# pbs-plus/pbs-plus

Measured on AMD Instinct MI355X. Metric: GiB/s ingested through CDC+SHA-256, higher is better.
Workload: dtype u32

## Files before the change

pbs_plus_amd/csrc/kernels.h:

```cpp
#pragma once

#include <hip/hip_runtime.h>
#include <stdint.h>

#include "../../include/pbsgpu.h"

namespace pbsk {

constexpr int kWindow = 64;

struct ScanParams {
    const uint8_t *data_al;
    uint32_t lead;
    uint64_t nbytes;
    uint64_t ntiles;
    uint32_t tile_bytes;
    const uint32_t *table_rot;
    uint32_t thr;
    uint32_t cap;
    uint32_t *tile_cnt;
    uint32_t *tile_slots;
    unsigned long long *tile_queue;
    uint32_t tiles_per_wave;
    uint32_t shared_chip;
// ... 159 lines not shown
    const uint4 *ldesc;
    uint32_t lmask;
    uint32_t long_bytes;
    const uint4 *sdesc;
    uint32_t smask;
    uint32_t short_bytes;
    uint32_t short_room;
    RingCtl *ctl;
    uint8_t *cells;
    uint32_t *pending;
    unsigned long long *free_fifo;
    uint32_t free_mask;
    const uint32_t *heartbeat;
    unsigned long long idle_ticks;
    uint32_t poll_mask;
    uint32_t xp;
    uint32_t long_spill;
    uint32_t xp_pairs;
    uint32_t long_lo;
};
constexpr int kHbBeat = 0, kHbIntent = 16, kHbCommitted = 17, kHbClaim = 32, kHbRoundsEnq = 33;
constexpr uint32_t kRingProbeSteps = 4096;


enum : int { kRsNcand = 0, kRsNrec = 1, kRsMaxcnt = 2, kRsNlong = 3, kRsNshort = 4, kRsShortRoom = 5, kRsTileq = 6 , kRsNmain = 8, kRsCount = 10 };

struct RingPage {
    uint64_t phys_off;
    uint64_t logical;
    uint32_t valid;
    uint32_t slot;
    uint32_t phys;
    uint32_t seg;
    uint64_t fill_seed;
    uint64_t fill_off;
    uint32_t fill_kind;
    uint32_t do_fill;
    const struct FillPiece *fill_tab;
    uint32_t fill_ntab;
    uint32_t prev_phys;
};
struct FillPiece {
    uint64_t dst_off, len, src_off, seed;
};
struct RingSeg {
    uint32_t slot;
    uint32_t first_page;
    uint32_t npages;
    uint32_t final;
    uint64_t new_end;
    uint32_t reset;
    uint32_t pad;
    uint64_t origin;
};
constexpr uint64_t kRingMaxStream = 1ull << kRingOffBits;
constexpr uint32_t kRingPT = 512;
struct RingStreamState {
    uint64_t c;
    uint64_t end;
    uint64_t ecand;
    uint32_t pad[2];
    uint32_t pt[kRingPT];
};
struct RingRoundStatus {
    uint32_t seq;
    uint32_t nrec;
    uint32_t ncand;
    uint32_t error;
    uint32_t tail;
    uint32_t pad[3];
    unsigned long long probe[6];
    uint32_t phase_ticks[6];
};
static_assert(sizeof(RingRoundStatus) == 104, "host slot: 128 bytes (ring.cpp: input_stride)");
struct RingRound {
    uint8_t *arena;
    uint32_t page_bytes, stride, tile_bytes, tpp;
// ... 7 lines not shown
    uint32_t seq;
    uint32_t cell_base, cell_cap, cell_mask;
    uint32_t scan_blocks;
    RingRoundStatus *status;
    RingStreamState *streams;
    RingSource q;
    uint4 *desc_w;
    uint4 *ldesc_w;
    uint4 *sdesc_w;
    unsigned long long *tile_queue;
    uint32_t *scalars;
    uint32_t *tile_cnt, *tile_off, *tile_slots, *scan_tmp;
    uint64_t *dense;
    uint64_t dense_cap;
    pbsgpu_segment *segs;
    uint32_t *seg_cnt, *seg_off;
    pbsgpu_record *recs;
    uint64_t rec_cap;
    uint64_t *seg_newc;
    uint32_t *seg_open;
    uint64_t *seg_ecand_in;
    uint64_t *seg_ecand;
    const uint64_t *sugg;
    const uint32_t *sugg_idx;
    uint64_t sugg_feed;
    uint32_t sugg_abs;
    uint32_t pad0;
    const uint32_t *seg_rec_base;
};
struct RingStage {
    const uint8_t *src;
    uint8_t *dst;
    uint32_t off[4], len[4];
    const RingPage *pages_host;
};
hipError_t launch_ring_round(const RingRound &r, int num_cus, hipStream_t st, hipStream_t fill_st = nullptr,
                             hipEvent_t fill_ev = nullptr, hipStream_t scan_st = nullptr, hipEvent_t scan_ev = nullptr,
                             const RingStage *stage = nullptr);
hipError_t launch_ring_service(const RingSource &q, unsigned workgroups, hipStream_t st, bool dense = false);
hipError_t launch_ring_service_xp(const RingSource &q, unsigned workgroups, hipStream_t st);
hipError_t launch_ring_service_lanes(const RingSource &q, unsigned workgroups, hipStream_t st, bool dense);
hipError_t launch_ring_stop(RingCtl *ctl, hipStream_t st);
hipError_t launch_ring_reset(RingCtl *ctl, hipStream_t st);

struct PackItem {
    uint64_t src_off;
    uint64_t dst_off;
    uint64_t len;
    uint32_t kind;
    uint32_t pad;
};
hipError_t launch_pack(const uint8_t *src_base, uint8_t *dst, const PackItem *items, uint32_t nitems, hipStream_t st);

}
```

pbs_plus_amd/csrc/ring.cpp:

```cpp
#include <chrono>
#include <cstdio>
#include <cstdlib>
#include <thread>

#include "ring_internal.h"

using namespace pbse;

namespace {

double now_ms() {
    return std::chrono::duration<double, std::milli>(std::chrono::steady_clock::now().time_since_epoch()).count();
}

uint32_t pow2_at_least(uint64_t v) {
    uint32_t p = 1;
    while (p < v && p < (1u << 31)) p <<= 1;
    return p;
}

volatile uint32_t *hb_words(const pbsgpu_ring *r) { return r->heartbeat.as<volatile uint32_t>(); }

void ring_service_ended(pbsgpu_ring *r) {
    if (r->svc == SvcState::Stopped) return;
// ... 135 lines not shown
int ring_start_service(pbsgpu_ring *r, bool force = false) {
    if (r->svc == SvcState::Running) return PBSGPU_OK;
    if (r->svc == SvcState::Stopping && r->parked_for_flush) {
        HIPCHK(hipStreamSynchronize(r->ss));
        ring_service_ended(r);
    }
    const uint32_t park_gen = service_park_generation(r->eng->device);
    if (r->svc == SvcState::Stopped && !force && park_gen != 0 && park_gen != r->park_grace_gen) {
        const double t = now_ms();
        if (r->park_wait_t0 == 0) r->park_wait_t0 = t;
        if (t - r->park_wait_t0 < 250.0) return PBSGPU_OK;
        r->park_grace_gen = park_gen;
    }
    r->park_wait_t0 = 0;
    if (r->svc == SvcState::Stopping) {
        HIPCHK(hipStreamWaitEvent(r->cs, r->ev_svc1, 0));
        HIPCHK(pbsk::launch_ring_reset(r->ctl.as<pbsk::RingCtl>(), r->cs));
        HIPCHK(hipEventRecord(r->ev_reset, r->cs));
    } else {
        service_started(r->eng->device);
    }
    r->svc = SvcState::Running;
    ring_adapt_split(r);
    r->defer_t0 = 0;
    hb_words(r)[pbsk::kHbClaim] = r->tail_seen;
    CHK(ring_launch_services(r));
    r->svc_t0 = now_ms();
    r->svc_bytes0 = r->st.bytes_enqueued - r->deferred_bytes;
    r->deferred_bytes = 0;
    r->st.service_launches++;
    return PBSGPU_OK;
}

int ring_enqueue_round(pbsgpu_ring *r, bool *did) {
    *did = false;
    pbsgpu_engine *e = r->eng;
    if (r->error != PBSGPU_OK) return r->error;
    bool any = false, any_final = false;
    size_t ready = 0;
    for (auto &s : r->slots) {
        if (!s.open) continue;
        any |= !s.ready.empty() || s.zero_final;
        any_final |= s.zero_final || (!s.ready.empty() && s.ready.back().final);
        ready += s.ready.size();
    }
    if (!any) return PBSGPU_OK;
    {
        size_t inflight = 0;
        for (auto &ri : r->rounds) inflight += ri.reaped ? 0 : 1;
        if (inflight > 0 && !any_final && ready < r->min_round_pages) return PBSGPU_OK;
        if (inflight >= r->max_inflight) return PBSGPU_OK;
    }
    int in = -1;
    for (uint32_t i = 0; i < kRingInputs; ++i)
        if (!r->input_busy[i]) { in = (int)i; break; }
    if (in < 0) return PBSGPU_OK;
    {
        const uint64_t oldest = r->rounds.empty() ? r->cell_cursor : r->rounds.front().cell_base;
        if (r->cell_cursor + r->rec_cap - oldest > r->ncells) return PBSGPU_OK;
    }
    pbsk::RingPage *pg = r->in_pages((uint32_t)in);
    pbsk::RingSeg *sg = r->in_segs((uint32_t)in);
    uint32_t *recbase = r->in_recbase((uint32_t)in);
    uint32_t *suggidx = r->in_suggidx((uint32_t)in);
    uint32_t np = 0, ns = 0;
    uint64_t cells_needed = 0, new_bytes = 0;
    RoundInfo ri;
    std::vector<hipEvent_t> deps;
    std::vector<uint64_t> sugg;
    const uint32_t minsz = std::min(e->effmin, e->cfg.min);
    const uint64_t feed = e->sugg_feed.load(std::memory_order_relaxed);
    const uint64_t look = feed > 1 ? (uint64_t)e->cfg.max : 0;
    uint32_t streams_waiting = 0;
    for (auto &s : r->slots) streams_waiting += (s.open && !s.ready.empty()) ? 1u : 0u;
    const uint32_t round_cap = (r->svc == SvcState::Stopped || streams_waiting < 2)
                                   ? r->round_pages
                                   : std::max(std::min(r->round_pages, r->min_round_pages), r->round_pages / 2);
    for (uint32_t si = 0; si < r->slots.size() && np < round_cap; ++si) {
        StreamSlot &s = r->slots[si];
        if (!s.open || (s.ready.empty() && !s.zero_final)) continue;
        pbsk::RingSeg g{};
        g.slot = si;
        g.first_page = np;
        g.reset = s.fresh ? 1u : 0u;
        g.origin = s.origin;
        const uint64_t end_old = s.bytes_enqueued;
        uint64_t end = end_old;
        uint32_t take = 0;
        while (!s.ready.empty() && take < kPagesPerStreamRound && np < round_cap) {
            const PageReq &q = s.ready.front();
            pbsk::RingPage p{};
            p.phys = q.phys;
            p.phys_off = (uint64_t)q.phys * r->stride + 128u;
            p.logical = ((uint64_t)si << pbsk::kRingOffBits) | (q.k * r->page_bytes);
            p.valid = q.valid;
            p.slot = si;
            p.seg = ns;
            p.do_fill = q.do_fill ? 1u : 0u;
            p.fill_seed = q.seed;
            p.fill_off = q.fill_off;
            p.fill_kind = q.kind;
            p.fill_tab = q.tab;
            p.fill_ntab = q.ntab;
            p.prev_phys = (q.k > 0 && s.last_phys >= 0) ? (uint32_t)s.last_phys : 0xffffffffu;
            s.last_phys = (int64_t)q.phys;
            pg[np++] = p;
            if (q.dep) deps.push_back(q.dep);
            end += q.valid;
            new_bytes += q.valid;
            if (q.final) g.final = 1;
            s.ready.pop_front();
            ++take;
        }
        if (s.zero_final && s.ready.empty()) {
            g.final = 1;
            s.zero_final = false;
        }
        g.npages = take;
        g.new_end = end;
        s.bytes_enqueued = end;
        s.fresh = false;
        if (g.final) {
            s.final_enqueued = true;
            ri.finals.push_back(si);
        }
        suggidx[ns] = (uint32_t)sugg.size();
        {
            const uint64_t lower = end_old > e->cfg.max ? end_old - e->cfg.max : 0;
            while (!s.sugg.empty() && s.sugg.front() < lower) s.sugg.pop_front();
            for (uint64_t b : s.sugg) {
                if (b > end + look) break;
                sugg.push_back(b);
            }
        }
        recbase[ns] = (uint32_t)cells_needed;
        cells_needed += ((uint64_t)take * r->page_bytes + e->cfg.max) / minsz + 2;
        sg[ns++] = g;
    }
    if (ns == 0) return PBSGPU_OK;
    suggidx[ns] = (uint32_t)sugg.size();
// ... 72 lines not shown
    rr.recs = r->recs.as<pbsgpu_record>();
    rr.rec_cap = r->rec_cap;
    rr.seg_newc = r->seg_newc.as<uint64_t>();
    rr.seg_open = r->seg_open.as<uint32_t>();
    rr.seg_ecand_in = r->seg_ecand_in.as<uint64_t>();
    rr.seg_ecand = r->seg_ecand.as<uint64_t>();
    rr.sugg = sugg_dev;
    rr.sugg_idx = sugg_dev ? suggidx : nullptr;
    rr.sugg_feed = feed;
    rr.sugg_abs = e->sugg_feed_abs.load(std::memory_order_relaxed);
    rr.seg_rec_base = recbase;
    std::atomic_thread_fence(std::memory_order_release);
    bool defer = r->defer_service;
    if (!defer && r->svc == SvcState::Stopped && r->lone_defer_ms > 0 && !any_final &&
        np >= std::max<uint32_t>(1, r->round_pages / 2)) {
        const uint64_t lanes_worth = (uint64_t)r->sha_cus * (r->dense_service ? 256u : 128u) * (uint64_t)e->cfg.avg;
        const double t = now_ms();
        if (r->defer_t0 == 0) r->defer_t0 = t;
        defer = t - r->defer_t0 < r->lone_defer_ms && r->deferred_bytes + new_bytes < lanes_worth;
    }
    if (!defer) {
        const int st = ring_start_service(r);
        if (st != PBSGPU_OK) return fail(st);
        rr.q = r->source();
    }
    if (r->svc == SvcState::Stopped) r->deferred_bytes += new_bytes;
    if (r->svc == SvcState::Stopped) rr.scan_blocks = (uint32_t)std::max(1, e->num_cus);
    else if (r->ps && rr.scan_blocks > 8) rr.scan_blocks -= 1;
    hipStream_t scan_st = r->ps ? r->ps : r->cs;
    for (hipEvent_t ev : deps)
        if (hipStreamWaitEvent(scan_st, ev, 0) != hipSuccess) return fail(PBSGPU_E_HIP);
    for (hipEvent_t ev : deps) ring_event_put(r, ev);
    deps.clear();
    if (r->ps && r->ctl_used[set])
        if (hipStreamWaitEvent(r->ps, r->ev_ctl[set], 0) != hipSuccess) return fail(PBSGPU_E_HIP);
    {
        const bool fill_serial = r->fill_serial;
        pbsk::RingStage stg{};
        if (r->stage_inputs) {
            const uint8_t *hb = r->in((uint32_t)in);
            uint8_t *db = r->in_dev((uint32_t)in);
            stg.src = hb;
            stg.dst = db;
            stg.off[0] = (uint32_t)r->in_pages_off;   stg.len[0] = np * (uint32_t)sizeof(pbsk::RingPage);
            stg.off[1] = (uint32_t)r->in_segs_off;    stg.len[1] = ns * (uint32_t)sizeof(pbsk::RingSeg);
            stg.off[2] = (uint32_t)r->in_recbase_off; stg.len[2] = (ns + 1u) * 4u;
            stg.off[3] = (uint32_t)r->in_suggidx_off; stg.len[3] = rr.sugg_idx ? (ns + 1u) * 4u : 0u;
            stg.pages_host = pg;
            auto mirror = [&](const void *hp) { return db + (reinterpret_cast<const uint8_t *>(hp) - hb); };
            rr.pages = reinterpret_cast<const pbsk::RingPage *>(mirror(pg));
            rr.segs_in = reinterpret_cast<const pbsk::RingSeg *>(mirror(sg));
            rr.seg_rec_base = reinterpret_cast<const uint32_t *>(mirror(recbase));
            if (rr.sugg_idx) rr.sugg_idx = reinterpret_cast<const uint32_t *>(mirror(suggidx));
        }
        const hipError_t he = pbsk::launch_ring_round(rr, e->num_cus, r->cs, fill_serial ? nullptr : r->fs, r->ev_fill[in], r->ps,
                                                      r->ps ? r->ev_scan[in] : nullptr, r->stage_inputs ? &stg : nullptr);
        if (he != hipSuccess) {
            g_last_hip_error.store((int)he);
            return fail(PBSGPU_E_HIP);
        }
    }
    if (r->ps) {
        if (hipEventRecord(r->ev_ctl[set], r->cs) != hipSuccess) return fail(PBSGPU_E_HIP);
        r->ctl_used[set] = true;
        r->scan_set ^= 1u;
    }
    r->input_busy[in] = true;
    ri.new_bytes = new_bytes;
    r->ready_bytes -= new_bytes;
    r->inflight_bytes += new_bytes;
    r->rounds.push_back(std::move(ri));
    r->st.rounds++;
    r->st.bytes_enqueued += new_bytes;
    r->st.pages_enqueued += np;
    *did = true;
    return PBSGPU_OK;
}

int ring_take_page(pbsgpu_ring *r, uint32_t *phys) {
    if (r->backlog_limit && r->svc == SvcState::Running) {
        const int32_t behind = (int32_t)(r->tail_seen - hb_words(r)[pbsk::kHbClaim]) - 256;
        double wait = (double)r->ready_bytes + (double)r->inflight_bytes;
        if (behind > 0 && r->pub_positions) wait += (double)behind * ((double)r->pub_bytes / (double)r->pub_positions);
        if (wait > (double)r->backlog_limit) return PBSGPU_E_BUSY;
    }
    if (r->free_pages.empty()) ring_reap_free(r);
    if (r->free_pages.empty()) return PBSGPU_E_BUSY;
    *phys = r->free_pages.back();
    r->free_pages.pop_back();
// ... 211 lines not shown
            arena_bytes = fr > (12ull << 30) ? fr - (8ull << 30) : fr / 2;
        }
        r->npages = (uint32_t)std::min<uint64_t>(arena_bytes / r->stride, 65534);
        {
            const uint64_t lim = (4ull << 20) * std::min(e->effmin, e->cfg.min) / r->page_bytes;
            if (r->npages > lim) r->npages = (uint32_t)std::max<uint64_t>(lim, 4);
        }
        if (r->npages < 4) return PBSGPU_E_INVALID;
        r->max_streams = o.max_streams ? o.max_streams : 64;
        if (r->max_streams > 4096) return PBSGPU_E_INVALID;
        int sha = o.sha_cus ? (int)o.sha_cus : std::max(1, e->num_cus - e->num_cus / 4);
        int xp = o.express_cus == PBSGPU_RING_OFF ? 0 : (int)o.express_cus;
        if (o.express_cus == 0 && !o.sha_cus && e->num_cus >= 128) xp = 16;
        xp = std::min(xp, std::max(0, e->num_cus / 2));
        if (xp && !o.sha_cus) sha = std::max(1, sha - xp);
        const int svc_max = std::max(2, e->num_cus - e->num_cus / 4 + (e->num_cus >= 64 ? 8 : 0));
        if (sha + xp > svc_max) sha = std::max(1, svc_max - xp);
        r->xp_cus = (uint32_t)xp;
        r->sha_cus = (uint32_t)std::min(std::max(sha, 1), std::max(1, e->num_cus - 1 - xp));
        r->lanes_cus = std::min<uint32_t>(o.lanes_cus, r->sha_cus * 3u / 4u);
        r->sha_cus -= r->lanes_cus;
        r->short_bytes = o.short_bytes ? (uint32_t)std::min<uint64_t>(o.short_bytes, e->cfg.max) : (uint32_t)((uint64_t)e->cfg.avg * 3 / 2);
        r->svc_cus = r->sha_cus + r->xp_cus + r->lanes_cus;
        r->split_auto = xp > 0 && !o.sha_cus && !o.express_cus && r->svc_cus >= 96 && !(o.flags & PBSGPU_RING_F_NO_SPLIT_AUTO);
        r->round_pages = o.round_pages ? o.round_pages : 256;
        r->round_pages = std::min(r->round_pages, r->npages);
        r->min_round_pages = o.min_round_pages ? std::max(1u, std::min(o.min_round_pages, std::max(1u, r->round_pages / 4)))
                                               : std::max(1u, r->round_pages / 4);
        r->backlog_limit = o.backlog_mib < 0 ? 0 : o.backlog_mib > 0 ? (uint64_t)(o.backlog_mib * 1048576.0)   : (uint64_t)(r->sha_cus + r->lanes_cus) << 27;
        r->backlog_auto = o.backlog_mib == 0;
        if (o.max_inflight) r->max_inflight = std::min<uint32_t>(std::max(1u, o.max_inflight), kRingInputs);
        r->autopark_ms = std::max(0.0, o.autopark_ms);
        r->defer_service = (o.flags & PBSGPU_RING_F_DEFER_SERVICE) != 0;
        r->fill_serial = (o.flags & PBSGPU_RING_F_FILL_SERIAL) != 0;
        r->dense_service = (o.flags & PBSGPU_RING_F_DENSE_SERVICE) != 0;
        r->dense_lanes = (o.flags & PBSGPU_RING_F_DENSE_LANES) != 0;
        r->tier_tag = (o.flags & PBSGPU_RING_F_TIER_TAG) != 0;
        r->lone_defer_ms = o.lone_defer_ms < 0 ? 0.0 : o.lone_defer_ms > 0 ? o.lone_defer_ms : 25.0;
        r->idle_timeout_s = o.idle_timeout_s;
        r->opt_long_lo = o.long_lo_bytes;
        r->opt_long_spill = o.long_spill;
        r->opt_poll_every = o.poll_every;
        const double lambda = 3.0 * r->tile_bytes / ((double)e->cfg.mask + 1.0);
        uint32_t capv = 8;
        while (capv < 4.0 * lambda + 16.0) capv <<= 1;
        r->cap = std::min<uint32_t>(std::max<uint32_t>(capv * 2, r->tile_bytes / 128), r->tile_bytes);
        const uint64_t ntiles = (uint64_t)r->round_pages * r->tpp;
        if (ntiles * r->cap >= (1ull << 32)) return PBSGPU_E_INVALID;
        const uint32_t minsz = std::min(e->effmin, e->cfg.min);
        r->dense_cap = ntiles * r->cap;
        r->rec_cap = ((uint64_t)r->round_pages * r->page_bytes + (uint64_t)r->max_streams * e->cfg.max) / minsz +
                     4ull * r->max_streams + 64;
        const uint64_t resident_chunks = (uint64_t)r->npages * r->page_bytes / minsz + 2ull * r->npages + r->rec_cap;
        r->qslots = pow2_at_least(2 * resident_chunks + 4096);
        r->ncells = pow2_at_least(4 * resident_chunks + 4 * r->rec_cap);
        r->nfree = pow2_at_least(4ull * r->npages + 64);

        CHK(r->arena.ensure((size_t)r->npages * r->stride + 512));
        CHK(r->ctl.ensure(256));
        CHK(r->probe.ensure(128));
        CHK(r->streams.ensure((size_t)r->max_streams * sizeof(pbsk::RingStreamState)));
        CHK(r->pending.ensure((size_t)r->npages * 4 + 64));
        CHK(r->desc.ensure((size_t)r->qslots * 32));
        r->long_bytes = r->xp_cus ? (long_bytes_hint ? long_bytes_hint : (uint32_t)((uint64_t)e->cfg.max * 13 / 16)) : 0;
        r->long_lo_auto = long_bytes_hint == 0;
        if (o.long_bytes) r->long_bytes = o.long_bytes == PBSGPU_RING_OFF ? 0u : o.long_bytes;
        if (r->xp_cus && r->long_bytes == 0) r->xp_cus = 0;
// ... 98 lines not shown
    return ring_create_internal(e, opt, true, out);
}

int pbsgpu_ring_quiesce(pbsgpu_ring *r) {
    if (!r) return PBSGPU_E_INVALID;
    CHK(set_device(r->eng));
    ring_heartbeat(r);
    if (r->defer_service && r->svc == SvcState::Stopped) {
        HIPCHK(hipStreamSynchronize(r->cs));
        HIPCHK(pbsk::launch_ring_stop(r->ctl.as<pbsk::RingCtl>(), r->cs));
        HIPCHK(hipEventRecord(r->ev_reset, r->cs));
        CHK(ring_launch_services(r));
        service_started(r->eng->device);
        r->svc = SvcState::Running;
        r->st.service_launches++;
        HIPCHK(hipStreamSynchronize(r->ss));
        ring_service_ended(r);
        HIPCHK(hipStreamSynchronize(r->cs));
        r->svc_bytes0 = r->st.bytes_enqueued;
        ring_reap_free(r);
        ring_reap_rounds(r);
        return r->error;
    }
    if (r->svc == SvcState::Stopped && r->deferred_bytes > 0) {
        CHK(ring_start_service(r, true));
    }
    if (r->svc == SvcState::Running) {
        CHK(ring_service_check(r, false));
        if (r->svc == SvcState::Running) HIPCHK(pbsk::launch_ring_stop(r->ctl.as<pbsk::RingCtl>(), r->cs));
    }
    HIPCHK(hipStreamSynchronize(r->cs));
    if (r->svc != SvcState::Stopped) {
        HIPCHK(hipStreamSynchronize(r->ss));
        HIPCHK(hipStreamSynchronize(r->fs));
        ring_service_ended(r);
    }
    ring_reap_free(r);
    ring_reap_rounds(r);
    return r->error;
}

int pbsgpu_ring_park(pbsgpu_ring *r) {
    if (!r) return PBSGPU_E_INVALID;
    CHK(set_device(r->eng));
    ring_heartbeat(r);
    CHK(ring_park(r));
    return r->error;
}

void pbsgpu_ring_destroy(pbsgpu_ring *r) {
    if (!r) return;
    pbsgpu_engine *e = r->eng;
    if (e) {
        (void)hipSetDevice(e->device);
        if (r->cs && r->ss) (void)pbsgpu_ring_quiesce(r);
        if (r->svc != SvcState::Stopped) {
            r->svc = SvcState::Stopped;
            service_ended(r->eng->device);
        }
        if (r->ss) (void)hipStreamDestroy(r->ss);
        if (r->xs) (void)hipStreamDestroy(r->xs);
        if (r->ev_xsvc1) (void)hipEventDestroy(r->ev_xsvc1);
        if (r->ls) (void)hipStreamDestroy(r->ls);
        if (r->ev_lsvc1) (void)hipEventDestroy(r->ev_lsvc1);
        if (r->cs) (void)hipStreamDestroy(r->cs);
        if (r->ps) (void)hipStreamDestroy(r->ps);
        if (r->fs) (void)hipStreamDestroy(r->fs);
        for (auto ev : r->ev_scan)
            if (ev) (void)hipEventDestroy(ev);
        for (auto ev : r->ev_ctl)
            if (ev) (void)hipEventDestroy(ev);
        for (auto ev : r->ev_fill)
            if (ev) (void)hipEventDestroy(ev);
        for (hipEvent_t ev : {r->ev_reset, r->ev_svc0, r->ev_svc1})
            if (ev) (void)hipEventDestroy(ev);
        for (auto &s : r->slots)
            for (auto &q : s.ready)
                if (q.dep) r->ev_pool.push_back(q.dep);
        for (auto ev : r->ev_pool) (void)hipEventDestroy(ev);
        for (DevBuf *b : {&r->arena, &r->ctl, &r->probe, &r->streams, &r->pending, &r->desc, &r->ldesc, &r->sdesc, &r->scalars, &r->tile_cnt, &r->tile_off,
                          &r->tile_slots, &r->tile_cnt2, &r->tile_slots2, &r->tileq, &r->scan_tmp, &r->dense, &r->segs, &r->seg_cnt, &r->seg_off, &r->recs, &r->seg_newc,
                          &r->seg_open, &r->seg_ecand_in, &r->seg_ecand, &r->inputs_dev})
            b->release();
        r->cells.release();
        r->heartbeat.release();
        r->free_fifo.release();
        r->inputs.release();
        for (auto &b : r->sugg_in) b.release();
// ... 208 lines not shown
    StreamSlot &s = r->slots[stream];
    if (s.final_committed) return PBSGPU_E_STATE;
    if (!s.sugg.empty() && offset < s.sugg.back()) return PBSGPU_E_INVALID;
    s.sugg.push_back(offset);
    return PBSGPU_OK;
}

int pbsgpu_ring_fill(pbsgpu_ring *r, uint32_t stream, uint64_t seed, uint32_t kind, uint64_t nbytes, int final,
                     uint64_t *taken) {
    if (!r || !taken || stream >= r->slots.size() || !r->slots[stream].open || kind > 4) return PBSGPU_E_INVALID;
    StreamSlot &s = r->slots[stream];
    *taken = 0;
    if (s.final_committed || s.reserved >= 0) return PBSGPU_E_STATE;
    if (r->error != PBSGPU_OK) return r->error;
    if (s.bytes_committed + nbytes > pbsk::kRingMaxStream) return PBSGPU_E_INVALID;
    if (nbytes == 0) {
        if (final) {
            s.zero_final = true;
            s.final_committed = true;
        }
        return PBSGPU_OK;
    }
    while (*taken < nbytes) {
        const uint64_t n = std::min<uint64_t>(r->page_bytes, nbytes - *taken);
        const bool last = (*taken + n == nbytes);
        if (n < r->page_bytes && !(last && final)) break;
        uint32_t phys = 0;
        if (ring_take_page(r, &phys) != PBSGPU_OK) break;
        PageReq q;
        q.phys = phys;
        q.k = s.next_k++;
        q.valid = (uint32_t)n;
        q.final = last && final;
        q.do_fill = true;
        q.seed = seed;
        q.kind = kind;
        q.fill_off = s.bytes_committed;
        if (r->hold) r->held.assign(stream, q.k, q.phys);
        s.ready.push_back(q);
        r->ready_bytes += n;
        s.bytes_committed += n;
        *taken += n;
        if (q.final) s.final_committed = true;
    }
    return PBSGPU_OK;
}

int pbsgpu_ring_fill_pieces(pbsgpu_ring *r, uint32_t stream, const pbsgpu_fill_piece *pieces, uint32_t npieces, uint64_t nbytes,
                            int final, uint64_t *taken) {
    if (!r || !taken || stream >= r->slots.size() || !r->slots[stream].open) return PBSGPU_E_INVALID;
    static_assert(sizeof(pbsgpu_fill_piece) == sizeof(pbsk::FillPiece), "piece layout");
    StreamSlot &s = r->slots[stream];
    *taken = 0;
    if (s.final_committed || s.reserved >= 0) return PBSGPU_E_STATE;
    if (r->error != PBSGPU_OK) return r->error;
    if (pieces) {
        if (npieces == 0 || s.bytes_committed != 0) return PBSGPU_E_INVALID;
        uint64_t pos = 0;
        for (uint32_t i = 0; i < npieces; ++i) {
            if (pieces[i].dst_off != pos || pieces[i].len == 0 || ((pieces[i].dst_off | pieces[i].len | pieces[i].src_off) & 15u))
                return PBSGPU_E_INVALID;
            pos += pieces[i].len;
        }
        CHK(r->piece_tab[stream].ensure(std::max<size_t>((size_t)npieces * sizeof(pbsk::FillPiece), 4096)));
        std::memcpy(r->piece_tab[stream].p, pieces, (size_t)npieces * sizeof(pbsk::FillPiece));
        r->piece_n[stream] = npieces;
    }
    const uint32_t nt = r->piece_n[stream];
    if (nt == 0) return PBSGPU_E_STATE;
    const pbsk::FillPiece *tab = r->piece_tab[stream].as<pbsk::FillPiece>();
    const uint64_t total = tab[nt - 1].dst_off + tab[nt - 1].len;
    if (s.bytes_committed + nbytes > total || s.bytes_committed + nbytes > pbsk::kRingMaxStream) return PBSGPU_E_INVALID;
    if (nbytes == 0) {
        if (final) {
            s.zero_final = true;
            s.final_committed = true;
        }
        return PBSGPU_OK;
    }
    while (*taken < nbytes) {
        const uint64_t n = std::min<uint64_t>(r->page_bytes, nbytes - *taken);
        const bool last = (*taken + n == nbytes);
        if (n < r->page_bytes && !(last && final)) break;
        uint32_t phys = 0;
        if (ring_take_page(r, &phys) != PBSGPU_OK) break;
        PageReq q;
        q.phys = phys;
        q.k = s.next_k++;
        q.valid = (uint32_t)n;
        q.final = last && final;
        q.do_fill = true;
        q.kind = 5;
        q.tab = tab;
        q.ntab = nt;
        q.fill_off = s.bytes_committed;
        if (r->hold) r->held.assign(stream, q.k, q.phys);
        s.ready.push_back(q);
        r->ready_bytes += n;
        s.bytes_committed += n;
        *taken += n;
        if (q.final) s.final_committed = true;
    }
    return PBSGPU_OK;
}

int pbsgpu_ring_pump(pbsgpu_ring *r) {
    if (!r) return PBSGPU_E_INVALID;
    CHK(set_device(r->eng));
    ring_heartbeat(r);
    CHK(ring_service_check(r, false));
    if (r->svc == SvcState::Stopping) {
        const hipError_t q = hipEventQuery(r->ev_svc1);
        if (q == hipSuccess) ring_service_ended(r);
        else (void)hipGetLastError();
    }
    ring_reap_free(r);
    ring_reap_rounds(r);
    if (r->svc == SvcState::Running) {
        const uint32_t gen = service_park_generation(r->eng->device);
        if (gen && gen != r->park_gen_seen) {
            r->park_gen_seen = gen;
            CHK(ring_park(r));
            if (r->svc == SvcState::Stopping) r->parked_for_flush = true;
        }
    }
    bool any_round = false;
    for (int i = 0; i < 4; ++i) {
        bool did = false;
        CHK(ring_enqueue_round(r, &did));
        if (!did) break;
        any_round = true;
    }
    if (!r->defer_service && r->svc == SvcState::Stopped && r->deferred_bytes > 0) {
        bool waiting = false;
        for (auto &s : r->slots) waiting |= s.open && !s.ready.empty();
        const uint64_t lanes_worth = (uint64_t)r->sha_cus * (r->dense_service ? 256u : 128u) * (uint64_t)r->eng->cfg.avg;
        if ((!any_round && !waiting) || now_ms() - r->defer_t0 >= r->lone_defer_ms || r->deferred_bytes >= lanes_worth)
            CHK(ring_start_service(r));
    }
    if (r->autopark_ms > 0 && r->svc == SvcState::Running) {
        if (ring_idle(r)) {
            const double t = now_ms();
// ... 138 lines not shown
```

pbs_plus_amd/csrc/ring_internal.h:

```cpp
#pragma once

#include <deque>
#include <mutex>
#include <vector>

#include "engine_internal.h"
#include "hold.h"

namespace pbse {

constexpr uint32_t kRingInputs = 16;
constexpr uint32_t kPagesPerStreamRound = 256;

struct PageReq {
    uint32_t phys = 0;
    uint64_t k = 0;
    uint32_t valid = 0;
    bool final = false;
    bool do_fill = false;
    uint64_t seed = 0, fill_off = 0;
    uint32_t kind = 0;
    const pbsk::FillPiece *tab = nullptr;
    uint32_t ntab = 0;
    hipEvent_t dep = nullptr;
};

struct CellRef {
    uint32_t cell;
    uint32_t round_idx;
};

struct StreamSlot {
    bool open = false;
    bool fresh = true;
    uint64_t next_k = 0;
    uint64_t bytes_committed = 0;
    uint64_t bytes_enqueued = 0;
    bool final_committed = false, final_enqueued = false, final_done = false;
    bool zero_final = false;
    int64_t reserved = -1;
    int64_t last_phys = -1;
    std::deque<PageReq> ready;
    std::deque<CellRef> cells;
    uint64_t records_out = 0;
    uint64_t polled_end = 0;
    bool reported = false;
    uint64_t origin = 0;
    std::deque<uint64_t> sugg;
    void *owner = nullptr;
};

struct RoundInfo {
    uint32_t seq = 0;
    uint32_t input = 0;
    uint64_t cell_base = 0;
    uint32_t cell_cap = 0;
// ... 23 lines not shown
    pbse::DevBuf arena, ctl, streams, pending, desc, ldesc, sdesc, probe;
    unsigned long long probe_seen[6] = {};
    bool probe_seen_valid = false;
    unsigned long long ctl_phase_ticks[2][5] = {};
    unsigned long long ctl_phase_rounds[2] = {};
    uint32_t lslots = 0, long_bytes = 0;
    uint32_t sslots = 0, short_bytes = 0, lanes_cus = 0;
    pbse::DevBuf scalars, tile_cnt, tile_off, tile_slots, scan_tmp, dense, segs, seg_cnt, seg_off, recs, seg_newc, seg_open;
    pbse::DevBuf tile_cnt2, tile_slots2, tileq;
    pbse::DevBuf seg_ecand_in, seg_ecand;
    pbse::DevBuf inputs_dev;
    bool stage_inputs = true;
    bool long_lo_auto = false;
    pbse::PinnedBuf cells, free_fifo, inputs, heartbeat;
    std::vector<pbse::PinnedBuf> piece_tab;
    std::vector<uint32_t> piece_n;
    pbse::PinnedBuf sugg_in[pbse::kRingInputs];
    size_t input_stride = 0, in_pages_off = 0, in_segs_off = 0, in_recbase_off = 0, in_suggidx_off = 0, in_status_off = 0;
    hipStream_t cs = nullptr, ss = nullptr, fs = nullptr;
    hipStream_t ls = nullptr;
    hipStream_t xs = nullptr;
    hipStream_t ps = nullptr;
    hipEvent_t ev_scan[pbse::kRingInputs] = {};
    hipEvent_t ev_ctl[2] = {};
    bool ctl_used[2] = {false, false};
    uint32_t scan_set = 0;
    int bulk_prio = 0;
    uint32_t xp_cus = 0;
    bool split_auto = false;
    uint32_t svc_cus = 0;
    double obs_bytes = 0, obs_long_bytes = 0;
    hipEvent_t ev_reset = nullptr, ev_svc0 = nullptr, ev_svc1 = nullptr, ev_xsvc1 = nullptr, ev_lsvc1 = nullptr;
    hipEvent_t ev_fill[pbse::kRingInputs] = {};
    std::vector<hipEvent_t> ev_pool;
    pbse::SvcState svc = pbse::SvcState::Stopped;
    uint32_t rounds_enq = 0;
    double autopark_ms = 0;
    double idle_since_ms = 0;
    bool dense_service = false;
    bool dense_lanes = false;
    bool tier_tag = false;
    bool backlog_auto = true;
    uint32_t park_gen_seen = 0;
    uint32_t park_grace_gen = 0;
    double park_wait_t0 = 0;
    bool parked_for_flush = false;
    bool fill_serial = false;
    bool hold = false;
    pbse::HeldPages held;
    uint32_t opt_long_lo = 0, opt_long_spill = 0, opt_poll_every = 0;
    bool defer_service = false;
    double lone_defer_ms = 25.0;
    double defer_t0 = 0;
    uint64_t deferred_bytes = 0;
    double idle_timeout_s = 0;
    std::vector<uint32_t> free_pages;
    uint32_t free_read = 0;
    std::vector<pbse::StreamSlot> slots;
    std::deque<pbse::RoundInfo> rounds;
    bool input_busy[pbse::kRingInputs] = {};
    uint32_t next_seq = 1;
    uint64_t cell_cursor = 0;
    int error = PBSGPU_OK;
    pbsgpu_ring_stats st{};
    double svc_t0 = 0;
    uint64_t svc_bytes0 = 0;

    uint8_t *in(uint32_t i) const { return inputs.as<uint8_t>() + (size_t)i * input_stride; }
    uint8_t *in_dev(uint32_t i) const { return inputs_dev.as<uint8_t>() + (size_t)i * input_stride; }
    pbsk::RingPage *in_pages(uint32_t i) const { return reinterpret_cast<pbsk::RingPage *>(in(i) + in_pages_off); }
    pbsk::RingSeg *in_segs(uint32_t i) const { return reinterpret_cast<pbsk::RingSeg *>(in(i) + in_segs_off); }
    uint32_t *in_recbase(uint32_t i) const { return reinterpret_cast<uint32_t *>(in(i) + in_recbase_off); }
    uint32_t *in_suggidx(uint32_t i) const { return reinterpret_cast<uint32_t *>(in(i) + in_suggidx_off); }
    pbsk::RingRoundStatus *in_status(uint32_t i) const {
        return reinterpret_cast<pbsk::RingRoundStatus *>(in(i) + in_status_off);
    }
    pbsk::RingSource source() const;
};

namespace pbse {
// ... 40 lines not shown
```

pbs_plus_amd/csrc/ring_kernels.inc:

```

__device__ __forceinline__ bool ring_short_ticket(const RingRound &r, const RingDesc &d) {
    const uint32_t idx = atomicAdd(&r.scalars[kRsNshort], 1u);
    if (idx >= r.scalars[kRsShortRoom]) return false;
    ring_desc_encode(r.sdesc_w, (r.q.ctl->stail + idx) & r.q.smask, d);
    return true;
}

__global__ __launch_bounds__(256) void k_ring_fill(RingRound r) {
    const RingPage &pe = r.pages[blockIdx.y];
    if (!pe.do_fill) return;
    uint64_t *dst = reinterpret_cast<uint64_t *>(r.arena + pe.phys_off);
    const uint64_t nwords = ((uint64_t)pe.valid + 7u) / 8u;
    const uint64_t w0 = pe.fill_off >> 3;
    const uint64_t stride = (uint64_t)gridDim.x * blockDim.x;
    if (pe.fill_kind == 4u) {
        uint4 *d4 = reinterpret_cast<uint4 *>(dst);
        const uint32_t nblk = (uint32_t)((nwords + 1u) / 2u), step = gridDim.x * blockDim.x;
        const uint64_t q0 = w0 >> 1;
        uint32_t i = blockIdx.x * blockDim.x + threadIdx.x;
        for (; i + 3u * step < nblk; i += 4u * step) {
            const uint4 a = chacha2_block(q0 + i, pe.fill_seed), b = chacha2_block(q0 + i + step, pe.fill_seed);
            const uint4 c = chacha2_block(q0 + i + 2u * step, pe.fill_seed), d = chacha2_block(q0 + i + 3u * step, pe.fill_seed);
            d4[i] = a;
            d4[i + step] = b;
            d4[i + 2u * step] = c;
            d4[i + 3u * step] = d;
        }
        for (; i < nblk; i += step) d4[i] = chacha2_block(q0 + i, pe.fill_seed);
        return;
    }
    if (pe.fill_kind == 5u) {
        uint4 *d4 = reinterpret_cast<uint4 *>(dst);
        const uint32_t nblk = (uint32_t)((nwords + 1u) / 2u), step = gridDim.x * blockDim.x;
        const FillPiece *tab = pe.fill_tab;
        const uint32_t nt = pe.fill_ntab;
        FillPiece pc{~0ull, 0, 0, 0};
        for (uint32_t i = blockIdx.x * blockDim.x + threadIdx.x; i < nblk; i += step) {
            const uint64_t x = pe.fill_off + 16ull * i;
            if (!(x >= pc.dst_off && x - pc.dst_off < pc.len)) {
                uint32_t lo = 0, hi = nt;
                while (hi - lo > 1u) {
                    const uint32_t mid = (lo + hi) >> 1;
                    if (tab[mid].dst_off <= x) lo = mid; else hi = mid;
                }
                pc = tab[lo];
            }
            d4[i] = chacha2_block((pc.src_off + (x - pc.dst_off)) >> 4, pc.seed);
        }
        return;
    }
    for (uint64_t i = (uint64_t)blockIdx.x * blockDim.x + threadIdx.x; i < nwords; i += stride)
        dst[i] = fill_word(w0 + i, pe.fill_seed, pe.fill_kind);
}

__global__ __launch_bounds__(64) void k_ring_prep_pages(RingRound r) {
    const uint32_t b = blockIdx.x;
    const int t = threadIdx.x;
    if (b == 0 && t == 0) *r.tile_queue = 0ull;
    if (b >= r.npages || t >= 8) return;
    const RingPage &pe = r.pages[b];
    uint4 v = make_uint4(0, 0, 0, 0);
    if (pe.prev_phys != 0xffffffffu)
        v = reinterpret_cast<const uint4 *>(r.arena + (uint64_t)pe.prev_phys * r.stride + 128u + r.page_bytes - 128)[t];
    reinterpret_cast<uint4 *>(r.arena + pe.phys_off - 128)[t] = v;
}

__global__ __launch_bounds__(64) void k_ring_prep(RingRound r) {
    const uint32_t b = blockIdx.x;
    const int t = threadIdx.x;
    if (b == 0 && t < kRsCount) {
        uint32_t v = 0;
        if (t == kRsShortRoom && r.q.short_bytes) {
            const unsigned long long sq = __hip_atomic_load(&r.q.ctl->sq, __ATOMIC_RELAXED, __HIP_MEMORY_SCOPE_AGENT);
            const uint32_t waiting = (uint32_t)sq - (uint32_t)(sq >> 32);
            v = waiting < r.q.short_room ? r.q.short_room - waiting : 0u;
        }
        r.scalars[t] = v;
    }
    if (b < r.npages) {
        const RingPage &pe = r.pages[b];
        const RingSeg &sg = r.segs_in[pe.seg];
        RingStreamState *st = r.streams + pe.slot;
        const uint64_t off = pe.logical & kRingOffMask;
        const uint64_t k = off / r.page_bytes;
        const uint8_t *body = r.arena + pe.phys_off;
// ... 297 lines not shown
    __syncthreads();
    if (tid == 0) {
        RingRoundStatus *hs = r.status;
        hs->phase_ticks[0] = (uint32_t)(tk1 - tk0);
        hs->phase_ticks[1] = (uint32_t)(tk2 - tk1);
        hs->phase_ticks[2] = (uint32_t)(tk3 - tk2);
        hs->phase_ticks[3] = (uint32_t)(tk4 - tk3);
        hs->phase_ticks[4] = (uint32_t)(wall_clock64() - tk4);
        hs->phase_ticks[5] = (uint32_t)tk0;
        ring_publish_tail(r, n_s, err);
    }
}

__global__ void k_ring_stop(RingCtl *ctl) { __hip_atomic_store(&ctl->stop, 1u, __ATOMIC_RELEASE, __HIP_MEMORY_SCOPE_AGENT); }

__global__ void k_ring_reset(RingCtl *ctl) {
    ctl->head = ctl->tail;
    ctl->lhead = ctl->ltail;
    ctl->xp_busy = 0;
    ctl->shead = ctl->stail;
    ctl->stop = 0;
}

hipError_t launch_ring_stop(RingCtl *ctl, hipStream_t st) {
    hipLaunchKernelGGL(k_ring_stop, dim3(1), dim3(1), 0, st, ctl);
    return hipGetLastError();
}

hipError_t launch_ring_reset(RingCtl *ctl, hipStream_t st) {
    hipLaunchKernelGGL(k_ring_reset, dim3(1), dim3(1), 0, st, ctl);
    return hipGetLastError();
}

constexpr unsigned kRingLdsTag = 1024;

__global__ __launch_bounds__(256) void k_ring_stage(RingStage s) {
    const uint32_t sp = blockIdx.y;
    const uint32_t n16 = (s.len[sp] + 15u) / 16u;
    const uint4 *a = reinterpret_cast<const uint4 *>(s.src + s.off[sp]);
    uint4 *b = reinterpret_cast<uint4 *>(s.dst + s.off[sp]);
    for (uint32_t i = blockIdx.x * blockDim.x + threadIdx.x; i < n16; i += gridDim.x * blockDim.x) b[i] = a[i];
}

hipError_t launch_ring_round(const RingRound &r, int num_cus, hipStream_t st, hipStream_t fill_st, hipEvent_t fill_ev,
                             hipStream_t scan_st, hipEvent_t scan_ev, const RingStage *stage) {
    hipStream_t sst = scan_st ? scan_st : st;
    bool any_fill = false;
    const RingPage *hp = stage ? stage->pages_host : r.pages;
    for (uint32_t i = 0; i < r.npages; ++i) any_fill |= hp[i].do_fill != 0;
    if (stage) {
        uint32_t mx = 1;
        for (int k = 0; k < 4; ++k) mx = std::max(mx, (stage->len[k] / 16u + 255u) / 256u);
        hipLaunchKernelGGL(k_ring_stage, dim3(std::min(mx, 8u), 4), dim3(256), kRingLdsTag, (any_fill && fill_st) ? fill_st : sst, *stage);
    }
    if (any_fill) {
        hipLaunchKernelGGL(k_ring_fill, dim3(16, r.npages), dim3(256), kRingLdsTag, fill_st ? fill_st : sst, r);
        if (fill_st && fill_st != sst) {
            hipError_t e = hipEventRecord(fill_ev, fill_st);
            if (e != hipSuccess) return e;
            e = hipStreamWaitEvent(sst, fill_ev, 0);
            if (e != hipSuccess) return e;
        }
    }
    hipLaunchKernelGGL(k_ring_prep_pages, dim3(r.npages ? r.npages : 1), dim3(64), kRingLdsTag, sst, r);
    const uint64_t ntiles = (uint64_t)r.npages * r.tpp;
    if (ntiles) {
        ScanParams p{};
        p.data_al = r.arena;
        p.lead = 0;
        p.nbytes = ~0ull >> 1;
        p.ntiles = ntiles;
        p.tile_bytes = r.tile_bytes;
        p.table_rot = r.table_rot;
        p.thr = r.thr;
        p.cap = r.cap;
        p.tile_cnt = r.tile_cnt;
        p.tile_slots = r.tile_slots;
        p.tile_queue = r.tile_queue;
        p.ring_pages = r.pages;
        p.ring_tpp = r.tpp;
        p.max_blocks = r.scan_blocks;
        hipError_t e = (r.tile_bytes == 64u * 34u * 128u) ? launch_scan3_any<34>(p, num_cus, sst) : launch_scan3_any<4>(p, num_cus, sst);
        if (e != hipSuccess) return e;
    }
    if (sst != st) {
        hipError_t e = hipEventRecord(scan_ev, sst);
        if (e != hipSuccess) return e;
        e = hipStreamWaitEvent(st, scan_ev, 0);
        if (e != hipSuccess) return e;
    }
    hipLaunchKernelGGL(k_ring_prep, dim3(r.npages + r.nseg), dim3(64), kRingLdsTag, st, r);
    hipLaunchKernelGGL(k_ring_control, dim3(1), dim3(1024), kRingLdsTag, st, r, SuggFeed{r.sugg_feed, 0, r.sugg_abs, 0});
    return hipGetLastError();
}

// ... 38 lines not shown
```

Measured before the change: 633.0.

## Decouple page fill from round launch into batched fill jobs on fill stream

Page fills (chacha/synthetic data generation) are no longer carried in RingPage and launched as part of each round. They are queued as RingFillJob entries when pages are submitted and flushed in batches of up to 64 on the fill stream, with the scan stream waiting on a fill event only when the round contains filled pages. This lets fills start earlier and overlap with the previous round's scan. It also shrinks RingPage and removes the host-side scan for any_fill. It adds a dependency on correct flush ordering and drops the serial-fill option.

```diff
diff --git a/pbs_plus_amd/csrc/kernels.h b/pbs_plus_amd/csrc/kernels.h
--- a/pbs_plus_amd/csrc/kernels.h
+++ b/pbs_plus_amd/csrc/kernels.h
@@ -215,17 +215,26 @@
     uint32_t slot;
     uint32_t phys;
     uint32_t seg;
-    uint64_t fill_seed;
-    uint64_t fill_off;
-    uint32_t fill_kind;
-    uint32_t do_fill;
-    const struct FillPiece *fill_tab;
-    uint32_t fill_ntab;
     uint32_t prev_phys;
 };
 struct FillPiece {
     uint64_t dst_off, len, src_off, seed;
 };
+struct RingFillJob {
+    uint8_t *body;
+    uint64_t off;
+    uint64_t seed;
+    const FillPiece *tab;
+    uint32_t ntab;
+    uint32_t valid;
+    uint32_t kind;
+    uint32_t pad;
+};
+constexpr uint32_t kRingFillJobs = 64;
+struct RingFillJobs {
+    RingFillJob j[kRingFillJobs];
+};
+hipError_t launch_ring_fill(const RingFillJob *jobs, uint32_t n, uint64_t page_bytes, hipStream_t st);
 struct RingSeg {
     uint32_t slot;
     uint32_t first_page;
@@ -299,11 +308,9 @@
     const uint8_t *src;
     uint8_t *dst;
     uint32_t off[4], len[4];
-    const RingPage *pages_host;
-};
-hipError_t launch_ring_round(const RingRound &r, int num_cus, hipStream_t st, hipStream_t fill_st = nullptr,
-                             hipEvent_t fill_ev = nullptr, hipStream_t scan_st = nullptr, hipEvent_t scan_ev = nullptr,
-                             const RingStage *stage = nullptr);
+};
+hipError_t launch_ring_round(const RingRound &r, int num_cus, hipStream_t st, hipStream_t scan_st = nullptr,
+                             hipEvent_t scan_ev = nullptr, const RingStage *stage = nullptr);
 hipError_t launch_ring_service(const RingSource &q, unsigned workgroups, hipStream_t st, bool dense = false);
 hipError_t launch_ring_service_xp(const RingSource &q, unsigned workgroups, hipStream_t st);
 hipError_t launch_ring_service_lanes(const RingSource &q, unsigned workgroups, hipStream_t st, bool dense);
diff --git a/pbs_plus_amd/csrc/ring.cpp b/pbs_plus_amd/csrc/ring.cpp
--- a/pbs_plus_amd/csrc/ring.cpp
+++ b/pbs_plus_amd/csrc/ring.cpp
@@ -191,10 +191,40 @@
     return PBSGPU_OK;
 }
 
+static void ring_queue_fill(pbsgpu_ring *r, PageReq &q, uint64_t off, uint64_t seed, uint32_t kind, const pbsk::FillPiece *tab,
+                            uint32_t ntab) {
+    pbsk::RingFillJob j{};
+    j.body = r->arena.as<uint8_t>() + (uint64_t)q.phys * r->stride + 128u;
+    j.off = off;
+    j.seed = seed;
+    j.tab = tab;
+    j.ntab = ntab;
+    j.valid = q.valid;
+    j.kind = kind;
+    r->fill_jobs.push_back(j);
+    q.filled = true;
+}
+
+static int ring_flush_fills(pbsgpu_ring *r) {
+    const size_t n = r->fill_jobs.size();
+    for (size_t i = 0; i < n; i += pbsk::kRingFillJobs) {
+        const uint32_t m = (uint32_t)std::min<size_t>(pbsk::kRingFillJobs, n - i);
+        const hipError_t he = pbsk::launch_ring_fill(r->fill_jobs.data() + i, m, r->page_bytes, r->fs);
+        if (he != hipSuccess) {
+            g_last_hip_error.store((int)he);
+            r->fill_jobs.clear();
+            return r->error = PBSGPU_E_HIP;
+        }
+    }
+    r->fill_jobs.clear();
+    return PBSGPU_OK;
+}
+
 int ring_enqueue_round(pbsgpu_ring *r, bool *did) {
     *did = false;
     pbsgpu_engine *e = r->eng;
     if (r->error != PBSGPU_OK) return r->error;
+    CHK(ring_flush_fills(r));
     bool any = false, any_final = false;
     size_t ready = 0;
     for (auto &s : r->slots) {
@@ -226,6 +256,7 @@
     uint64_t cells_needed = 0, new_bytes = 0;
     RoundInfo ri;
     std::vector<hipEvent_t> deps;
+    bool any_filled = false;
     std::vector<uint64_t> sugg;
     const uint32_t minsz = std::min(e->effmin, e->cfg.min);
     const uint64_t feed = e->sugg_feed.load(std::memory_order_relaxed);
@@ -255,16 +286,11 @@
             p.valid = q.valid;
             p.slot = si;
             p.seg = ns;
-            p.do_fill = q.do_fill ? 1u : 0u;
-            p.fill_seed = q.seed;
-            p.fill_off = q.fill_off;
-            p.fill_kind = q.kind;
-            p.fill_tab = q.tab;
-            p.fill_ntab = q.ntab;
             p.prev_phys = (q.k > 0 && s.last_phys >= 0) ? (uint32_t)s.last_phys : 0xffffffffu;
             s.last_phys = (int64_t)q.phys;
             pg[np++] = p;
             if (q.dep) deps.push_back(q.dep);
+            any_filled |= q.filled;
             end += q.valid;
             new_bytes += q.valid;
             if (q.final) g.final = 1;
@@ -403,10 +429,13 @@
         if (hipStreamWaitEvent(scan_st, ev, 0) != hipSuccess) return fail(PBSGPU_E_HIP);
     for (hipEvent_t ev : deps) ring_event_put(r, ev);
     deps.clear();
+    if (any_filled) {
+        if (hipEventRecord(r->ev_fill[in], r->fs) != hipSuccess) return fail(PBSGPU_E_HIP);
+        if (hipStreamWaitEvent(scan_st, r->ev_fill[in], 0) != hipSuccess) return fail(PBSGPU_E_HIP);
+    }
     if (r->ps && r->ctl_used[set])
         if (hipStreamWaitEvent(r->ps, r->ev_ctl[set], 0) != hipSuccess) return fail(PBSGPU_E_HIP);
     {
-        const bool fill_serial = r->fill_serial;
         pbsk::RingStage stg{};
         if (r->stage_inputs) {
             const uint8_t *hb = r->in((uint32_t)in);
@@ -417,15 +446,14 @@
             stg.off[1] = (uint32_t)r->in_segs_off;    stg.len[1] = ns * (uint32_t)sizeof(pbsk::RingSeg);
             stg.off[2] = (uint32_t)r->in_recbase_off; stg.len[2] = (ns + 1u) * 4u;
             stg.off[3] = (uint32_t)r->in_suggidx_off; stg.len[3] = rr.sugg_idx ? (ns + 1u) * 4u : 0u;
-            stg.pages_host = pg;
             auto mirror = [&](const void *hp) { return db + (reinterpret_cast<const uint8_t *>(hp) - hb); };
             rr.pages = reinterpret_cast<const pbsk::RingPage *>(mirror(pg));
             rr.segs_in = reinterpret_cast<const pbsk::RingSeg *>(mirror(sg));
             rr.seg_rec_base = reinterpret_cast<const uint32_t *>(mirror(recbase));
             if (rr.sugg_idx) rr.sugg_idx = reinterpret_cast<const uint32_t *>(mirror(suggidx));
         }
-        const hipError_t he = pbsk::launch_ring_round(rr, e->num_cus, r->cs, fill_serial ? nullptr : r->fs, r->ev_fill[in], r->ps,
-                                                      r->ps ? r->ev_scan[in] : nullptr, r->stage_inputs ? &stg : nullptr);
+        const hipError_t he = pbsk::launch_ring_round(rr, e->num_cus, r->cs, r->ps, r->ps ? r->ev_scan[in] : nullptr,
+                                                      r->stage_inputs ? &stg : nullptr);
         if (he != hipSuccess) {
             g_last_hip_error.store((int)he);
             return fail(PBSGPU_E_HIP);
@@ -703,7 +731,6 @@
         if (o.max_inflight) r->max_inflight = std::min<uint32_t>(std::max(1u, o.max_inflight), kRingInputs);
         r->autopark_ms = std::max(0.0, o.autopark_ms);
         r->defer_service = (o.flags & PBSGPU_RING_F_DEFER_SERVICE) != 0;
-        r->fill_serial = (o.flags & PBSGPU_RING_F_FILL_SERIAL) != 0;
         r->dense_service = (o.flags & PBSGPU_RING_F_DENSE_SERVICE) != 0;
         r->dense_lanes = (o.flags & PBSGPU_RING_F_DENSE_LANES) != 0;
         r->tier_tag = (o.flags & PBSGPU_RING_F_TIER_TAG) != 0;
@@ -868,9 +895,10 @@
     HIPCHK(hipStreamSynchronize(r->cs));
     if (r->svc != SvcState::Stopped) {
         HIPCHK(hipStreamSynchronize(r->ss));
-        HIPCHK(hipStreamSynchronize(r->fs));
         ring_service_ended(r);
     }
+    if (r->error == PBSGPU_OK) CHK(ring_flush_fills(r));
+    HIPCHK(hipStreamSynchronize(r->fs));
     ring_reap_free(r);
     ring_reap_rounds(r);
     return r->error;
@@ -890,6 +918,7 @@
     if (e) {
         (void)hipSetDevice(e->device);
         if (r->cs && r->ss) (void)pbsgpu_ring_quiesce(r);
+        if (r->fs) (void)hipStreamSynchronize(r->fs);
         if (r->svc != SvcState::Stopped) {
             r->svc = SvcState::Stopped;
             service_ended(r->eng->device);
@@ -1164,10 +1193,7 @@
         q.k = s.next_k++;
         q.valid = (uint32_t)n;
         q.final = last && final;
-        q.do_fill = true;
-        q.seed = seed;
-        q.kind = kind;
-        q.fill_off = s.bytes_committed;
+        ring_queue_fill(r, q, s.bytes_committed, seed, kind, nullptr, 0);
         if (r->hold) r->held.assign(stream, q.k, q.phys);
         s.ready.push_back(q);
         r->ready_bytes += n;
@@ -1221,11 +1247,7 @@
         q.k = s.next_k++;
         q.valid = (uint32_t)n;
         q.final = last && final;
-        q.do_fill = true;
-        q.kind = 5;
-        q.tab = tab;
-        q.ntab = nt;
-        q.fill_off = s.bytes_committed;
+        ring_queue_fill(r, q, s.bytes_committed, 0, 5, tab, nt);
         if (r->hold) r->held.assign(stream, q.k, q.phys);
         s.ready.push_back(q);
         r->ready_bytes += n;
@@ -1240,6 +1262,7 @@
     if (!r) return PBSGPU_E_INVALID;
     CHK(set_device(r->eng));
     ring_heartbeat(r);
+    if (r->error == PBSGPU_OK) CHK(ring_flush_fills(r));
     CHK(ring_service_check(r, false));
     if (r->svc == SvcState::Stopping) {
         const hipError_t q = hipEventQuery(r->ev_svc1);
diff --git a/pbs_plus_amd/csrc/ring_internal.h b/pbs_plus_amd/csrc/ring_internal.h
--- a/pbs_plus_amd/csrc/ring_internal.h
+++ b/pbs_plus_amd/csrc/ring_internal.h
@@ -17,11 +17,7 @@
     uint64_t k = 0;
     uint32_t valid = 0;
     bool final = false;
-    bool do_fill = false;
-    uint64_t seed = 0, fill_off = 0;
-    uint32_t kind = 0;
-    const pbsk::FillPiece *tab = nullptr;
-    uint32_t ntab = 0;
+    bool filled = false;
     hipEvent_t dep = nullptr;
 };
 
@@ -111,6 +107,7 @@
     double obs_bytes = 0, obs_long_bytes = 0;
     hipEvent_t ev_reset = nullptr, ev_svc0 = nullptr, ev_svc1 = nullptr, ev_xsvc1 = nullptr, ev_lsvc1 = nullptr;
     hipEvent_t ev_fill[pbse::kRingInputs] = {};
+    std::vector<pbsk::RingFillJob> fill_jobs;
     std::vector<hipEvent_t> ev_pool;
     pbse::SvcState svc = pbse::SvcState::Stopped;
     uint32_t rounds_enq = 0;
@@ -124,7 +121,6 @@
     uint32_t park_grace_gen = 0;
     double park_wait_t0 = 0;
     bool parked_for_flush = false;
-    bool fill_serial = false;
     bool hold = false;
     pbse::HeldPages held;
     uint32_t opt_long_lo = 0, opt_long_spill = 0, opt_poll_every = 0;
diff --git a/pbs_plus_amd/csrc/ring_kernels.inc b/pbs_plus_amd/csrc/ring_kernels.inc
--- a/pbs_plus_amd/csrc/ring_kernels.inc
+++ b/pbs_plus_amd/csrc/ring_kernels.inc
@@ -6,37 +6,37 @@
     return true;
 }
 
-__global__ __launch_bounds__(256) void k_ring_fill(RingRound r) {
-    const RingPage &pe = r.pages[blockIdx.y];
-    if (!pe.do_fill) return;
-    uint64_t *dst = reinterpret_cast<uint64_t *>(r.arena + pe.phys_off);
-    const uint64_t nwords = ((uint64_t)pe.valid + 7u) / 8u;
-    const uint64_t w0 = pe.fill_off >> 3;
-    const uint64_t stride = (uint64_t)gridDim.x * blockDim.x;
-    if (pe.fill_kind == 4u) {
+constexpr unsigned kRingLdsTag = 1024;
+
+__device__ __forceinline__ void ring_fill_page(const RingFillJob &j, uint32_t bx, uint32_t nx) {
+    uint64_t *dst = reinterpret_cast<uint64_t *>(j.body);
+    const uint64_t nwords = ((uint64_t)j.valid + 7u) / 8u;
+    const uint64_t w0 = j.off >> 3;
+    const uint64_t stride = (uint64_t)nx * blockDim.x;
+    if (j.kind == 4u) {
         uint4 *d4 = reinterpret_cast<uint4 *>(dst);
-        const uint32_t nblk = (uint32_t)((nwords + 1u) / 2u), step = gridDim.x * blockDim.x;
+        const uint32_t nblk = (uint32_t)((nwords + 1u) / 2u), step = nx * blockDim.x;
         const uint64_t q0 = w0 >> 1;
-        uint32_t i = blockIdx.x * blockDim.x + threadIdx.x;
+        uint32_t i = bx * blockDim.x + threadIdx.x;
         for (; i + 3u * step < nblk; i += 4u * step) {
-            const uint4 a = chacha2_block(q0 + i, pe.fill_seed), b = chacha2_block(q0 + i + step, pe.fill_seed);
-            const uint4 c = chacha2_block(q0 + i + 2u * step, pe.fill_seed), d = chacha2_block(q0 + i + 3u * step, pe.fill_seed);
+            const uint4 a = chacha2_block(q0 + i, j.seed), b = chacha2_block(q0 + i + step, j.seed);
+            const uint4 c = chacha2_block(q0 + i + 2u * step, j.seed), d = chacha2_block(q0 + i + 3u * step, j.seed);
             d4[i] = a;
             d4[i + step] = b;
             d4[i + 2u * step] = c;
             d4[i + 3u * step] = d;
         }
-        for (; i < nblk; i += step) d4[i] = chacha2_block(q0 + i, pe.fill_seed);
+        for (; i < nblk; i += step) d4[i] = chacha2_block(q0 + i, j.seed);
         return;
     }
-    if (pe.fill_kind == 5u) {
+    if (j.kind == 5u) {
         uint4 *d4 = reinterpret_cast<uint4 *>(dst);
-        const uint32_t nblk = (uint32_t)((nwords + 1u) / 2u), step = gridDim.x * blockDim.x;
-        const FillPiece *tab = pe.fill_tab;
-        const uint32_t nt = pe.fill_ntab;
+        const uint32_t nblk = (uint32_t)((nwords + 1u) / 2u), step = nx * blockDim.x;
+        const FillPiece *tab = j.tab;
+        const uint32_t nt = j.ntab;
         FillPiece pc{~0ull, 0, 0, 0};
-        for (uint32_t i = blockIdx.x * blockDim.x + threadIdx.x; i < nblk; i += step) {
-            const uint64_t x = pe.fill_off + 16ull * i;
+        for (uint32_t i = bx * blockDim.x + threadIdx.x; i < nblk; i += step) {
+            const uint64_t x = j.off + 16ull * i;
             if (!(x >= pc.dst_off && x - pc.dst_off < pc.len)) {
                 uint32_t lo = 0, hi = nt;
                 while (hi - lo > 1u) {
@@ -49,8 +49,20 @@
         }
         return;
     }
-    for (uint64_t i = (uint64_t)blockIdx.x * blockDim.x + threadIdx.x; i < nwords; i += stride)
-        dst[i] = fill_word(w0 + i, pe.fill_seed, pe.fill_kind);
+    for (uint64_t i = (uint64_t)bx * blockDim.x + threadIdx.x; i < nwords; i += stride)
+        dst[i] = fill_word(w0 + i, j.seed, j.kind);
+}
+
+__global__ __launch_bounds__(256) void k_ring_fill(RingFillJobs a) { ring_fill_page(a.j[blockIdx.y], blockIdx.x, gridDim.x); }
+
+hipError_t launch_ring_fill(const RingFillJob *jobs, uint32_t n, uint64_t page_bytes, hipStream_t st) {
+    if (n == 0 || n > kRingFillJobs) return hipErrorInvalidValue;
+    RingFillJobs a{};
+    for (uint32_t i = 0; i < n; ++i) a.j[i] = jobs[i];
+    const uint32_t by_count = 1024u / n, by_size = (uint32_t)std::min<uint64_t>(page_bytes / (16u * 256u * 4u), 1024u);
+    const uint32_t gx = std::max(16u, std::min(by_count, by_size));
+    hipLaunchKernelGGL(k_ring_fill, dim3(gx, n), dim3(256), kRingLdsTag, st, a);
+    return hipGetLastError();
 }
 
 __global__ __launch_bounds__(64) void k_ring_prep_pages(RingRound r) {
@@ -414,8 +426,6 @@
     return hipGetLastError();
 }
 
-constexpr unsigned kRingLdsTag = 1024;
-
 __global__ __launch_bounds__(256) void k_ring_stage(RingStage s) {
     const uint32_t sp = blockIdx.y;
     const uint32_t n16 = (s.len[sp] + 15u) / 16u;
@@ -424,25 +434,13 @@
     for (uint32_t i = blockIdx.x * blockDim.x + threadIdx.x; i < n16; i += gridDim.x * blockDim.x) b[i] = a[i];
 }
 
-hipError_t launch_ring_round(const RingRound &r, int num_cus, hipStream_t st, hipStream_t fill_st, hipEvent_t fill_ev,
-                             hipStream_t scan_st, hipEvent_t scan_ev, const RingStage *stage) {
+hipError_t launch_ring_round(const RingRound &r, int num_cus, hipStream_t st, hipStream_t scan_st, hipEvent_t scan_ev,
+                             const RingStage *stage) {
     hipStream_t sst = scan_st ? scan_st : st;
-    bool any_fill = false;
-    const RingPage *hp = stage ? stage->pages_host : r.pages;
-    for (uint32_t i = 0; i < r.npages; ++i) any_fill |= hp[i].do_fill != 0;
     if (stage) {
         uint32_t mx = 1;
         for (int k = 0; k < 4; ++k) mx = std::max(mx, (stage->len[k] / 16u + 255u) / 256u);
-        hipLaunchKernelGGL(k_ring_stage, dim3(std::min(mx, 8u), 4), dim3(256), kRingLdsTag, (any_fill && fill_st) ? fill_st : sst, *stage);
-    }
-    if (any_fill) {
-        hipLaunchKernelGGL(k_ring_fill, dim3(16, r.npages), dim3(256), kRingLdsTag, fill_st ? fill_st : sst, r);
-        if (fill_st && fill_st != sst) {
-            hipError_t e = hipEventRecord(fill_ev, fill_st);
-            if (e != hipSuccess) return e;
-            e = hipStreamWaitEvent(sst, fill_ev, 0);
-            if (e != hipSuccess) return e;
-        }
+        hipLaunchKernelGGL(k_ring_stage, dim3(std::min(mx, 8u), 4), dim3(256), kRingLdsTag, sst, *stage);
     }
     hipLaunchKernelGGL(k_ring_prep_pages, dim3(r.npages ? r.npages : 1), dim3(64), kRingLdsTag, sst, r);
     const uint64_t ntiles = (uint64_t)r.npages * r.tpp;
```

After: 585.2. 0.924x the previous value.
